# Cyan4973/FiniteStateEntropy

Hardware: NVIDIA H100
Metric: encode+decode GB/s (uncompressed) per GPU on 32 KB blocks; bit-exact vs ref (higher is better)
Workload: dtype u8

## Files before the change

finitestateentropy_b200/csrc/huf_build_dev.cuh:

```cuda
#pragma once
#include "common.cuh"
#include "fse_dev.cuh"
#include "sink_dev.cuh"

namespace fseb {

struct HNode { u32 count; u16 parent; u8 sym; u8 len; };

__device__ inline u32 d_huf_limit_depth(HNode* nd, u32 last, u32 maxBits)
{
    u32 const deepest = nd[last].len;
    if (deepest <= maxBits) return deepest;
    int debt = 0;
    u32 const unit = 1u << (deepest - maxBits);
    int n = (int)last;
    u32 const NONE = 0xF0F0F0F0u;
    u32 lastOfRank[HUF_MAX_TLOG + 2];
    while (nd[n].len > maxBits) {
        debt += (int)(unit - (1u << (deepest - nd[n].len)));
        nd[n].len = (u8)maxBits; n--;
    }
    while (nd[n].len == maxBits) n--;
    debt >>= (deepest - maxBits);
    for (u32 i = 0; i < HUF_MAX_TLOG + 2; i++) lastOfRank[i] = NONE;
    {   u32 cur = maxBits;
        for (int pos = n; pos >= 0; pos--) {
            if (nd[pos].len >= cur) continue;
            cur = nd[pos].len;
            lastOfRank[maxBits - cur] = (u32)pos;
        }
    }
    while (debt > 0) {
        u32 dec = hibit((u32)debt) + 1;
        for (; dec > 1; dec--) {
            u32 const hi = lastOfRank[dec], lo = lastOfRank[dec - 1];
            if (hi == NONE) continue;
            if (lo == NONE) break;
            if (nd[hi].count <= 2 * nd[lo].count) break;
        }
        while (dec <= HUF_MAX_TLOG && lastOfRank[dec] == NONE) dec++;
        debt -= 1 << (dec - 1);
        if (lastOfRank[dec - 1] == NONE) lastOfRank[dec - 1] = lastOfRank[dec];
        nd[lastOfRank[dec]].len++;
        if (lastOfRank[dec] == 0) lastOfRank[dec] = NONE;
        else {
            lastOfRank[dec]--;
            if (nd[lastOfRank[dec]].len != maxBits - dec) lastOfRank[dec] = NONE;
        }
    }
    while (debt < 0) {
        if (lastOfRank[1] == NONE) {
            while (nd[n].len == maxBits) n--;
            nd[n + 1].len--;
            lastOfRank[1] = (u32)(n + 1);
            debt++;
            continue;
        }
        nd[lastOfRank[1] + 1].len--;
        lastOfRank[1]++;
        debt++;
    }
    return maxBits;
}

__device__ inline u64 cta_huf_build_ctable(u32* ctable, const u32* count, u32 msv, u32 maxBits,
                                           HNode* store, u32* lenOf, u32* firstVal)
{
    int const tid = threadIdx.x;
    HNode* const nd = store + 1;
    __shared__ u32 s_ret;
    if (!maxBits) maxBits = HUF_DEF_TLOG;
    if (msv > HUF_MAX_SV) return err(E_MSV_TOO_LARGE);
    for (int i = tid; i < 2 * 256 + 2; i += blockDim.x) { HNode z; z.count = 0; z.parent = 0; z.sym = 0; z.len = 0; store[i] = z; }
    __syncthreads();
    if ((u32)tid <= msv) {
        u32 const c = count[tid];
        u32 rank = 0;
        for (u32 jj = 0; jj <= msv; jj++) { u32 const cj = count[jj]; rank += (cj > c) | ((cj == c) & (jj < (u32)tid)); }
        nd[rank].count = c; nd[rank].sym = (u8)tid;
    }
    __syncthreads();
    if (tid == 0) {
        int last = (int)msv; while (nd[last].count == 0) last--;
        int fresh = 256, leaf = last, root = fresh + leaf - 1, inner = fresh;
        nd[fresh].count = nd[leaf].count + nd[leaf - 1].count;
        nd[leaf].parent = nd[leaf - 1].parent = (u16)fresh;
        fresh++; leaf -= 2;
        for (int n = fresh; n <= root; n++) nd[n].count = 1u << 30;
        nd[-1].count = 1u << 31;
        while (fresh <= root) {
            int const a = (nd[leaf].count < nd[inner].count) ? leaf-- : inner++;
            int const b = (nd[leaf].count < nd[inner].count) ? leaf-- : inner++;
            nd[fresh].count = nd[a].count + nd[b].count;
            nd[a].parent = nd[b].parent = (u16)fresh;
            fresh++;
        }
        nd[root].len = 0;
        for (int n = root - 1; n >= 256; n--) nd[n].len = (u8)(nd[nd[n].parent].len + 1);
        for (int n = 0; n <= last; n++) nd[n].len = (u8)(nd[nd[n].parent].len + 1);
        u32 const mb = d_huf_limit_depth(nd, (u32)last, maxBits);
        s_ret = mb;
        if (mb <= HUF_MAX_TLOG) {
            u32 perLen[HUF_MAX_TLOG + 1];
            for (u32 i = 0; i <= HUF_MAX_TLOG; i++) perLen[i] = 0;
            for (int n = 0; n <= last; n++) perLen[nd[n].len]++;
            u32 v = 0;
            for (u32 i = 0; i <= HUF_MAX_TLOG; i++) firstVal[i] = 0;
            for (int n = (int)mb; n > 0; n--) { firstVal[n] = v; v = (v + perLen[n]) >> 1; }
        }
    }
    __syncthreads();
    u32 const mb = s_ret;
    if (mb > HUF_MAX_TLOG) return err(E_GENERIC);
    if ((u32)tid <= msv) lenOf[nd[tid].sym] = nd[tid].len;
    __syncthreads();
    if ((u32)tid <= msv) {
        u32 const len = lenOf[tid];
        u32 before = 0;
        for (u32 jj = 0; jj < (u32)tid; jj++) before += (lenOf[jj] == len);
        ctable[tid] = ((firstVal[len] + before) & 0xFFFF) | (len << 16);
    } else ctable[tid & 255] = 0;
    __syncthreads();
    return mb;
}

__device__ __forceinline__ void warp_sort256_desc(u32 (&key)[8], unsigned lane)
{
    #pragma unroll
    for (u32 k = 2; k <= 256; k <<= 1) {
        #pragma unroll
        for (u32 j = k >> 1; j > 0; j >>= 1) {
            if (j >= 32) {
                u32 const dj = j >> 5;
                #pragma unroll
                for (u32 i = 0; i < 8; i++) {
                    if (i & dj) continue;
                    u32 const e = i * 32;
                    bool const desc = (k == 256) || ((e & k) != 0) ;
                    u32 const lo = min(key[i], key[i | dj]), hi = max(key[i], key[i | dj]);
                    key[i] = desc ? hi : lo; key[i | dj] = desc ? lo : hi;
                }
            } else {
                #pragma unroll
                for (u32 i = 0; i < 8; i++) {
                    u32 const e = i * 32 + lane;
                    u32 const other = __shfl_xor_sync(0xFFFFFFFFu, key[i], j);
                    bool const asc = (k == 256) ? false : ((e & k) == 0);
                    bool const takeMin = ((e & j) == 0) == asc;
                    key[i] = takeMin ? min(key[i], other) : max(key[i], other);
                }
            }
        }
    }
}

__device__ inline u64 warp_huf_build_ctable(u32* ctable, const u32* count, u32 msv, u32 maxBits,
                                            HNode* store, u8* lenOf, u32* firstVal)
{
    unsigned const lane = threadIdx.x & 31u;
    HNode* const nd = store + 1;
    if (!maxBits) maxBits = HUF_DEF_TLOG;
    if (msv > HUF_MAX_SV) return err(E_MSV_TOO_LARGE);
    {
        u32 key[8];
        #pragma unroll
        for (u32 i = 0; i < 8; i++) { u32 const s = i * 32 + lane; key[i] = ((s <= msv ? count[s] : 0u) << 8) | (255u - s); }
        warp_sort256_desc(key, lane);
        u64* const z = reinterpret_cast<u64*>(store);
        #pragma unroll
        for (u32 i = 0; i < 8; i++) {
            HNode h; h.count = key[i] >> 8; h.parent = 0; h.sym = (u8)(255u - (key[i] & 0xFFu)); h.len = 0;
            nd[i * 32 + lane] = h;
        }
        if (lane == 0) z[0] = 0;
        for (u32 i = 257 + lane; i < 2 * 256 + 2; i += 32) z[i] = 0;
    }
    __syncwarp();
    u32 mb = 0; int last = 0;
    if (lane == 0) {
        last = (int)msv; while (nd[last].count == 0) last--;
        int fresh = 256, leaf = last, root = fresh + leaf - 1, inner = fresh;
        nd[fresh].count = nd[leaf].count + nd[leaf - 1].count;
        nd[leaf].parent = nd[leaf - 1].parent = (u16)fresh;
        fresh++; leaf -= 2;
        for (int n = fresh; n <= root; n++) nd[n].count = 1u << 30;
        nd[-1].count = 1u << 31;
        u32 cl = nd[leaf].count, ci = nd[inner].count;
        while (fresh <= root) {
            int a, b2; u32 ca, cb;
            if (cl < ci) { a = leaf--; ca = cl; cl = nd[leaf].count; } else { a = inner++; ca = ci; ci = nd[inner].count; }
            if (cl < ci) { b2 = leaf--; cb = cl; cl = nd[leaf].count; } else { b2 = inner++; cb = ci; ci = nd[inner].count; }
            nd[fresh].count = ca + cb;
            if (inner == fresh) ci = ca + cb;
            nd[a].parent = nd[b2].parent = (u16)fresh;
            fresh++;
        }
        nd[root].len = 0;
        for (int n = root - 1; n >= 256; n--) nd[n].len = (u8)(nd[nd[n].parent].len + 1);
    }
    last = __shfl_sync(0xFFFFFFFFu, last, 0);
    __syncwarp();
    for (int n = (int)lane; n <= last; n += 32) nd[n].len = (u8)(nd[nd[n].parent].len + 1);
    __syncwarp();
    if (lane == 0) {
        mb = d_huf_limit_depth(nd, (u32)last, maxBits);
        if (mb <= HUF_MAX_TLOG) {
            u32 perLen[HUF_MAX_TLOG + 1];
            for (u32 i = 0; i <= HUF_MAX_TLOG; i++) perLen[i] = 0;
            for (int n = 0; n <= last; n++) perLen[nd[n].len]++;
            u32 v = 0;
            for (u32 i = 0; i <= HUF_MAX_TLOG; i++) firstVal[i] = 0;
            for (int n = (int)mb; n > 0; n--) { firstVal[n] = v; v = (v + perLen[n]) >> 1; }
        }
    }
    mb = __shfl_sync(0xFFFFFFFFu, mb, 0);
    if (mb > HUF_MAX_TLOG) return err(E_GENERIC);
    if (lane < 16) firstVal[16 + lane] = 0;
    __syncwarp();
    for (u32 s = lane; s <= msv; s += 32) lenOf[nd[s].sym] = nd[s].len;
    __syncwarp();
    u32* const seen = firstVal + 16;
    for (u32 s0 = 0; s0 < 256; s0 += 32) {
        u32 const s = s0 + lane;
        u32 const len = s <= msv ? lenOf[s] : 31u;
        u32 const peers = __match_any_sync(0xFFFFFFFFu, len);
        u32 val = 0;
        if (s <= msv) val = ((firstVal[len] + seen[len] + __popc(peers & ((1u << lane) - 1))) & 0xFFFF) | (len << 16);
        __syncwarp();
        if (s <= msv && (peers >> lane) == 1u) seen[len] += __popc(peers);
        ctable[s] = val;
        __syncwarp();
    }
    return mb;
}

__device__ inline u64 d_huf_compress_weights(u8* out, u64 cap, const u8* w, u64 n, u32* wksp)
{
    unsigned* const count = wksp;
    short* const norm = (short*)(wksp + 16);
    u32* const ct = wksp + 24;
    u16* const cellSym = (u16*)(wksp + 84);
    u32* const start = wksp + 116;
    unsigned msv = HUF_MAX_TLOG, tl = 6, best = 0;
    if (n <= 1) return 0;
    for (unsigned i = 0; i <= HUF_MAX_TLOG; i++) count[i] = 0;
    for (u64 i = 0; i < n; i++) count[w[i]]++;
    while (!count[msv]) msv--;
    for (unsigned s = 0; s <= msv; s++) best = count[s] > best ? count[s] : best;
    if (best == n) return 1;
    if (best == 1) return 0;
    tl = d_optimal_tablelog(tl, n, msv, 2);
    u64 r = d_normalize(norm, tl, count, n, msv); if (is_err(r)) return r;
    r = d_write_ncount(out, cap, norm, msv, tl); if (is_err(r)) return r;
    u64 const o = r;
    d_build_ctable_serial(ct, norm, msv, tl, cellSym, start);
    r = d_fse_encode_serial(out + o, cap - o, w, n, ct);
    if (r == 0) return 0;
    return o + r;
}

__device__ inline u64 d_huf_write_ctable(u8* out, u64 cap, const u32* ctable, unsigned msv, unsigned huffLog, u32* wksp)
{
    u8* const weight = (u8*)(wksp + 160);
    if (msv > HUF_MAX_SV) return err(E_MSV_TOO_LARGE);
    for (unsigned n = 0; n < msv; n++) {
        unsigned const len = (ctable[n] >> 16) & 0xFF;
        weight[n] = (u8)(len ? huffLog + 1 - len : 0);
    }
    {   u64 const h = d_huf_compress_weights(out + 1, cap - 1, weight, msv, wksp);
        if (is_err(h)) return h;
        if ((h > 1) & (h < msv / 2)) { out[0] = (u8)h; return h + 1; }
    }
    if (msv > 128) return err(E_GENERIC);
    if (((msv + 1) / 2) + 1 > cap) return err(E_DST_TOO_SMALL);
    out[0] = (u8)(128 + (msv - 1));
    weight[msv] = 0;
    for (unsigned n = 0; n < msv; n += 2) out[(n / 2) + 1] = (u8)((weight[n] << 4) + weight[n + 1]);
    return ((msv + 1) / 2) + 1;
}

__device__ inline u64 warp_huf_compress_weights(u8* out, u64 cap, const u8* w, u32 n, u32* wksp)
{
    unsigned const lane = threadIdx.x & 31u;
    unsigned* const count = wksp;
    short* const norm = (short*)(wksp + 16);
    u32* const ct = wksp + 24;
    u16* const cellSym = (u16*)(wksp + 84);
    u32* const start = wksp + 116;
    u16* const rec = (u16*)(wksp + 224);
    if (n <= 1) return 0;
    if (lane < 16) count[lane] = 0;
    __syncwarp();
    for (u32 i = lane; i < n; i += 32) atomicAdd(&count[w[i]], 1u);
    __syncwarp();
    unsigned msv = HUF_MAX_TLOG, best = 0;
    while (!count[msv]) msv--;
    for (unsigned s = 0; s <= msv; s++) best = count[s] > best ? count[s] : best;
    if (best == n) return 1;
    if (best == 1) return 0;
    unsigned const tl = d_optimal_tablelog(6, n, msv, 2);
    u64 r = 0;
    if (lane == 0) {
        r = d_normalize(norm, tl, count, n, msv);
        if (!is_err(r)) r = d_write_ncount(out, cap, norm, msv, tl);
        if (!is_err(r)) d_build_ctable_serial(ct, norm, msv, tl, cellSym, start);
    }
    r = __shfl_sync(0xFFFFFFFFu, r, 0);
    if (is_err(r)) return r;
    u32 const o = (u32)r;
    __syncwarp();
    if (n <= 2) return 0;
    u64 const scap = cap - o;
    if (scap <= 8) return 0;
    CtView const c = ct_view(ct);
    u32 state = 0;
    if (lane < 2) {
        bool seeded = false;
        int const first = (int)(((n - 1) & 1u) == lane ? n - 1 : n - 2);
        for (int i = first; i >= 0; i -= 2) {
            u32 const sym = w[i];
            if (!seeded) { state = enc_seed(c, sym); seeded = true; rec[i] = 0; }
            else {
                u32 const nb = (state + c.tt[2 * sym + 1]) >> 16;
                rec[i] = (u16)((state & ((1u << nb) - 1)) | (nb << 8));
                state = c.next[(state >> nb) + c.tt[2 * sym]];
            }
        }
    }
    u32 const s0 = __shfl_sync(0xFFFFFFFFu, state, 0), s1 = __shfl_sync(0xFFFFFFFFu, state, 1);
    for (u32 i = o + lane; i < (u32)cap; i += 32) out[i] = 0;
    __syncwarp();
    u64 const a0 = reinterpret_cast<u64>(out + o);
    u32* const words = reinterpret_cast<u32*>(a0 & ~3ull);
    u32 const limitWords = (u32)(((a0 & 3) + scap + 3) / 4);
    u32 running = 8 * (u32)(a0 & 3);
    u32 const bit0 = running;
    u32 const R = n + 3;
    for (u32 k0 = 0; k0 < R; k0 += 32) {
        u32 const k = k0 + lane;
        u32 e = 0;
        if (k < n) e = rec[n - 1 - k];
        else if (k == n) e = (s1 & ((1u << tl) - 1)) | (tl << 8);
        else if (k == n + 1) e = (s0 & ((1u << tl) - 1)) | (tl << 8);
        else if (k == n + 2) e = 1u | (1u << 8);
        u32 const nb = e >> 8, val = e & 0xFF;
        u32 incl = nb;
        #pragma unroll
        for (int d = 1; d < 32; d <<= 1) { u32 const t = __shfl_up_sync(0xFFFFFFFFu, incl, d); if (lane >= (unsigned)d) incl += t; }
        u32 const sum = __shfl_sync(0xFFFFFFFFu, incl, 31);
        if (nb) {
            u32 const off = running + incl - nb;
            u32 const wi = off >> 5, sh = off & 31;
            if (wi < limitWords) atomicOr(&words[wi], val << sh);
            if (sh + nb > 32 && wi + 1 < limitWords) atomicOr(&words[wi + 1], val >> (32 - sh));
        }
        running += sum;
    }
    __syncwarp();
    u32 const totalBits = running - bit0;
    if ((u64)(totalBits >> 3) >= scap - 8) return 0;
    return (u64)o + ((totalBits + 7) >> 3);
}

__device__ inline u64 warp_huf_write_ctable(u8* out, u64 cap, const u32* ctable, unsigned msv, unsigned huffLog, u32* wksp)
{
    unsigned const lane = threadIdx.x & 31u;
    u8* const weight = (u8*)(wksp + 160);
    if (msv > HUF_MAX_SV) return err(E_MSV_TOO_LARGE);
    for (unsigned n = lane; n < msv; n += 32) {
        unsigned const len = (ctable[n] >> 16) & 0xFF;
        weight[n] = (u8)(len ? huffLog + 1 - len : 0);
    }
    __syncwarp();
    {   u64 const h = warp_huf_compress_weights(out + 1, cap - 1, weight, msv, wksp);
        if (is_err(h)) return h;
        if ((h > 1) & (h < msv / 2)) { if (lane == 0) out[0] = (u8)h; __syncwarp(); return h + 1; }
    }
    if (msv > 128) return err(E_GENERIC);
    if (((msv + 1) / 2) + 1 > cap) return err(E_DST_TOO_SMALL);
    __syncwarp();
    if (lane == 0) { out[0] = (u8)(128 + (msv - 1)); weight[msv] = 0; }
    __syncwarp();
    for (unsigned n = 2 * lane; n < msv; n += 64) out[(n / 2) + 1] = (u8)((weight[n] << 4) + weight[n + 1]);
    __syncwarp();
    return ((msv + 1) / 2) + 1;
}

}
```

finitestateentropy_b200/csrc/huf_encode.cu:

```cuda
#include <cstdlib>
#include <mutex>
#include <vector>
#include "common.cuh"
#include "launch_util.cuh"
#include "fse_dev.cuh"
#include "sink_dev.cuh"
#include "huf_build_dev.cuh"

namespace fseb {
namespace hufe {

constexpr unsigned FULL = 0xFFFFFFFFu;

struct __align__(16) Plan {
    u32 ctable[256];
    u8  header[136];
    u32 hSize;
    u32 state;
    u32 total;
    u32 streamOff[4];
    u32 streamBytes[4];
};

constexpr int PLAN_WARPS = 8;
struct PlanWarp {
    u32   count4[4][256];
    u32   count[256];
    HNode nodes[2 * 256 + 2];
    u32   ctable[256];
    u32   firstVal[32];
    u8    lenOf[256];
    alignas(4) u8 header[136];
};
static_assert(sizeof(HNode) * (2 * 256 + 2) >= 384 * sizeof(u32), "header scratch must fit in the node array");
__device__ __forceinline__ u32 seg_count(const PlanWarp& w, u32 k, u32 i) { return w.count4[k][i]; }

__device__ __forceinline__ void warp_hist_range(u32* cnt, const u8* s, u32 begin, u32 end, unsigned lane)
{
    u32 i = begin;
    u32 const head = min(end, (u32)((begin + 15) & ~15u));
    bool const vec = ((reinterpret_cast<u64>(s) & 15) == 0);
    if (vec) {
        for (u32 k = i + lane; k < head; k += 32) atomicAdd(&cnt[s[k]], 1u);
        i = head;
        u32 const nvec = (end - i) / 16;
        const uint4* const gv = reinterpret_cast<const uint4*>(s + i);
        for (u32 v0 = 0; v0 < nvec; v0 += 128) {
            uint4 x[4];
            #pragma unroll
            for (int h = 0; h < 4; h++) { u32 const vi = v0 + 32 * h + lane; x[h] = (vi < nvec) ? __ldg(gv + vi) : make_uint4(0, 0, 0, 0); }
            #pragma unroll
            for (int h = 0; h < 4; h++) {
                if (v0 + 32 * h + lane >= nvec) continue;
                u32 const wd[4] = { x[h].x, x[h].y, x[h].z, x[h].w };
                #pragma unroll
                for (int k = 0; k < 4; k++) {
                    u32 const y = wd[k];
                    atomicAdd(&cnt[y & 0xFF], 1u); atomicAdd(&cnt[__byte_perm(y, 0, 0x4441)], 1u);
                    atomicAdd(&cnt[__byte_perm(y, 0, 0x4442)], 1u); atomicAdd(&cnt[y >> 24], 1u);
                }
            }
        }
        i += nvec * 16;
    }
    for (u32 k = i + lane; k < end; k += 32) atomicAdd(&cnt[s[k]], 1u);
}

__device__ __forceinline__ void warp_hist4_pipelined(u32 (*count4)[256], const u8* s, u32 n, u32 seg, unsigned lane)
{
    const uint4* const gv = reinterpret_cast<const uint4*>(s) + lane;
    u32 const B = n / 2048, perSeg = seg / 2048;
    auto load = [&](uint4 (&x)[4], u32 b) {
        #pragma unroll
        for (int h = 0; h < 4; h++) x[h] = __ldg(gv + b * 128 + 32 * h);
    };
    auto count = [&](const uint4 (&x)[4], u32 b) {
        u32* const cnt = count4[b / perSeg];
        #pragma unroll
        for (int h = 0; h < 4; h++) {
            u32 const wd[4] = { x[h].x, x[h].y, x[h].z, x[h].w };
            #pragma unroll
            for (int k = 0; k < 4; k++) {
                u32 const y = wd[k];
                atomicAdd(&cnt[y & 0xFF], 1u); atomicAdd(&cnt[__byte_perm(y, 0, 0x4441)], 1u);
                atomicAdd(&cnt[__byte_perm(y, 0, 0x4442)], 1u); atomicAdd(&cnt[y >> 24], 1u);
            }
        }
    };
    uint4 xa[4], xb[4];
    load(xa, 0);
    #pragma unroll 1
    for (u32 b = 0; b < B; b += 2) {
        if (b + 1 < B) load(xb, b + 1);
        count(xa, b);
        if (b + 2 < B) load(xa, b + 2);
        if (b + 1 < B) count(xb, b + 1);
    }
}

__global__ void __launch_bounds__(32 * PLAN_WARPS)
huf_plan_kernel(BatchGeom g, u8* __restrict__ cbuf, u64* __restrict__ csizes, const u8* __restrict__ src,
                unsigned msvReq, unsigned tlogReq, Plan* __restrict__ plans, int serialHeader)
{
    extern __shared__ __align__(16) unsigned char smem_raw[];
    PlanWarp& w = reinterpret_cast<PlanWarp*>(smem_raw)[threadIdx.x >> 5];
    unsigned const lane = threadIdx.x & 31u;
    u32 const b = blockIdx.x * PLAN_WARPS + (threadIdx.x >> 5);
    if (b >= g.nBlocks) return;
    u32 const n = block_len(g, b);
    const u8* const s = src + (u64)b * g.blockSize;
    u8* const d = cbuf + (u64)b * g.slot;
    u64 const cap = g.slot;
    Plan& P = plans[b];
#define FSEB_FINAL(v) do { if (lane == 0) { P.state = 1; csizes[b] = (v); } return; } while (0)

    if (!n) FSEB_FINAL(0);
    if (!cap) FSEB_FINAL(0);
    if (n > HUF_BLOCK_MAX) FSEB_FINAL(err(E_SRC_WRONG));
    if (tlogReq > HUF_MAX_TLOG) FSEB_FINAL(err(E_TLOG_TOO_LARGE));
    if (msvReq > HUF_MAX_SV) FSEB_FINAL(err(E_MSV_TOO_LARGE));
    unsigned const msvDecl = msvReq ? msvReq : HUF_MAX_SV;
    unsigned huffLog = tlogReq ? tlogReq : HUF_DEF_TLOG;

    u32 const seg = (n + 3) / 4;
    for (u32 i = lane; i < 4 * 256; i += 32) (&w.count4[0][0])[i] = 0;
    __syncwarp();
    if ((reinterpret_cast<u64>(s) & 15) == 0 && seg % 2048 == 0 && n == 4 * seg) warp_hist4_pipelined(w.count4, s, n, seg, lane);
    else {
        #pragma unroll 1
        for (u32 k = 0; k < 4; k++) {
            u32 const beg = min(k * seg, n), end = (k < 3) ? min((k + 1) * seg, n) : n;
            warp_hist_range(w.count4[k], s, beg, end, lane);
        }
    }
    __syncwarp();
    u32 top = 0, best = 0;
    for (u32 i = lane; i < 256; i += 32) {
        u32 const c = seg_count(w, 0, i) + seg_count(w, 1, i) + seg_count(w, 2, i) + seg_count(w, 3, i);
        w.count[i] = c;
        if (c) top = i; best = c > best ? c : best;
    }
    #pragma unroll
    for (int dlt = 16; dlt; dlt >>= 1) { top = max(top, __shfl_xor_sync(FULL, top, dlt)); best = max(best, __shfl_xor_sync(FULL, best, dlt)); }
    __syncwarp();
    if (msvDecl < 255 && top > msvDecl) FSEB_FINAL(err(E_MSV_TOO_SMALL));
    if (best == n) { if (lane == 0) d[0] = s[0]; FSEB_FINAL(1); }
    if (best <= (n >> 7) + 4) FSEB_FINAL(0);
    u32 const msv = top;

    huffLog = d_optimal_tablelog(huffLog, n, msv, 1);
    {   u64 const mb = warp_huf_build_ctable(w.ctable, w.count, msv, huffLog, w.nodes, w.lenOf, w.firstVal);
        if (is_err(mb)) FSEB_FINAL(mb);
        huffLog = (u32)mb;
    }
    __syncwarp();
    u32* const wksp = reinterpret_cast<u32*>(w.nodes);
    u64 hs = 0;
    if (serialHeader) { if (lane == 0) hs = d_huf_write_ctable(w.header, cap < sizeof(w.header) ? cap : sizeof(w.header), w.ctable, msv, huffLog, wksp); hs = __shfl_sync(FULL, hs, 0); }
    else hs = warp_huf_write_ctable(w.header, cap < sizeof(w.header) ? cap : sizeof(w.header), w.ctable, msv, huffLog, wksp);
    if (is_err(hs)) FSEB_FINAL(hs);
    if (hs + 12 >= n) FSEB_FINAL(0);
    u64 const capLeft = cap - hs;
    if (capLeft < 6 + 1 + 1 + 1 + 8 || n < 12) FSEB_FINAL(0);
    u32 bits[4];
    #pragma unroll
    for (int k = 0; k < 4; k++) {
        u32 acc = 0;
        for (u32 i = lane; i <= msv; i += 32) acc += seg_count(w, k, i) * (w.ctable[i] >> 16);
        #pragma unroll
        for (int dlt = 16; dlt; dlt >>= 1) acc += __shfl_xor_sync(FULL, acc, dlt);
        bits[k] = acc;
    }
    u64 op = 6; bool fits = true;
    u32 offs[4], lens[4];
    #pragma unroll
    for (int t = 0; t < 4; t++) {
        u64 const capk = capLeft - op;
        u64 const tot = (u64)bits[t] + 1;
        if (fits && (capk <= 8 || (tot >> 3) >= capk - 8)) fits = false;
        offs[t] = (u32)(hs + op); lens[t] = (u32)((tot + 7) >> 3);
        op += lens[t];
    }
    u64 const total = hs + op;
    if (!fits || total >= (u64)n - 1) FSEB_FINAL(0);
    __syncwarp();
    for (u32 i = lane; i < 256; i += 32) P.ctable[i] = w.ctable[i];
    for (u32 i = lane; i < (u32)hs; i += 32) P.header[i] = w.header[i];
    if (lane < 4) { P.streamOff[lane] = offs[lane]; P.streamBytes[lane] = lens[lane]; }
    if (lane == 0) { P.hSize = (u32)hs; P.state = 0; P.total = (u32)total; csizes[b] = total; }
#undef FSEB_FINAL
}

constexpr int THREADS = 128;

__device__ __noinline__ void store_piece_exact(u32* gw, u32 j, uint4 v, u32 a0, u32 endByte)
{
    u32 const wd[4] = { v.x, v.y, v.z, v.w };
    u8* const pb = reinterpret_cast<u8*>(gw + j);
    for (u32 t = 0; t < 16; t++) { u32 const at = 4 * j + t; if (at >= a0 && at < endByte) pb[t] = (u8)(wd[t >> 2] >> (8 * (t & 3))); }
}

__global__ void __launch_bounds__(THREADS)
huf_emit_kernel(BatchGeom g, u8* __restrict__ cbuf, const u8* __restrict__ src, const Plan* __restrict__ plans, const u32* __restrict__ sharedCT)
{
    constexpr u32 W = 512;
    __shared__ u32 ctab[256];
    constexpr u32 WP = W + 4;
    __shared__ __align__(16) u32 winAll[4 * WP];
    int const tid = threadIdx.x;
    unsigned const lane = tid & 31u; int const k = tid >> 5;
    u32 const b = blockIdx.x;
    const Plan& P = plans[b];
    if (P.state != 0) return;
    u32 const n = block_len(g, b);
    const u8* const s = src + (u64)b * g.blockSize;
    u8* const d = cbuf + (u64)b * g.slot;
    u32 const hSize = P.hSize, total = P.total;

    {   const u32* const ct = sharedCT ? sharedCT : P.ctable;
        u32 const c0 = ct[tid], c1 = ct[tid + 128];
        ctab[tid] = (c0 >> 16) | (c0 << 8 & 0xFFFF00u); ctab[tid + 128] = (c1 >> 16) | (c1 << 8 & 0xFFFF00u);
    }
    for (u32 i = tid; i < 4 * WP; i += THREADS) winAll[i] = 0;
    for (u32 i = tid; i < hSize; i += THREADS) d[i] = P.header[i];
    if (tid < 3) { u32 const v = P.streamBytes[tid]; d[hSize + 2 * tid] = (u8)v; d[hSize + 2 * tid + 1] = (u8)(v >> 8); }
    __syncthreads();
    {
        u32 const seg = (n + 3) / 4;
        int const segBeg = (int)(k * seg);
        int const segEnd = (k < 3) ? (int)((k + 1) * seg) : (int)n;
        u32 sTab = (u32)__cvta_generic_to_shared(ctab);
        asm volatile("mov.u32 %0, %0;" : "+r"(sTab));
        u32* const win = winAll + k * WP;
        u32 sWin = (u32)__cvta_generic_to_shared(win);
        asm volatile("mov.u32 %0, %0;" : "+r"(sWin));
        u8* const gstart = d + P.streamOff[k];
        u32 const a0 = (u32)(reinterpret_cast<u64>(gstart) & 15);
        u32* const gw = reinterpret_cast<u32*>(gstart - a0);
        u32 const sBytes = (k < 3) ? P.streamBytes[k] : total - P.streamOff[3];
        u32 const endByte = a0 + sBytes;
        u32 bitpos = 8u * a0;
        u32 flushed = 0;
// ... 199 lines not shown
    for (int t = 0; t < 4; t++) {
        u64 const capk = cap - op;
        u64 const tot = (u64)bits[t] + 1;
        if (fits && (capk <= 8 || (tot >> 3) >= capk - 8)) fits = false;
        offs[t] = (u32)op; lens[t] = (u32)((tot + 7) >> 3);
        op += lens[t];
    }
    if (!fits) { if (lane == 0) { P.state = 1; csizes[b] = 0; } return; }
    if (lane < 4) { P.streamOff[lane] = offs[lane]; P.streamBytes[lane] = lens[lane]; }
    if (lane == 0) { P.hSize = 0; P.state = 0; P.total = (u32)op; csizes[b] = op; }
}

}

cudaError_t launch_huf_encode_using_ctable(const BatchGeom& g, void* cbuf, u64* csizes, const void* src, const u32* dCTable, cudaStream_t stream)
{
    if (g.nBlocks == 0) return cudaSuccess;
    cudaError_t e;
    hufe::Plan* const plans = (hufe::Plan*)stream_scratch(2, stream, sizeof(hufe::Plan) * (size_t)g.nBlocks, &e);
    if (e != cudaSuccess) return e;
    unsigned const grid = (g.nBlocks + hufe::PLAN_WARPS - 1) / hufe::PLAN_WARPS;
    hufe::huf_sizes_kernel<<<grid, 32 * hufe::PLAN_WARPS, 0, stream>>>(g, csizes, (const u8*)src, dCTable, plans);
    hufe::huf_emit_kernel<<<g.nBlocks, hufe::THREADS, 0, stream>>>(g, (u8*)cbuf, (const u8*)src, plans, dCTable);
    return cudaGetLastError();
}

cudaError_t launch_huf_encode(const BatchGeom& g, void* cbuf, u64* csizes, const void* src,
                              unsigned msv, unsigned tlog, cudaStream_t stream)
{
    if (g.nBlocks == 0) return cudaSuccess;
    cudaError_t e;
    hufe::Plan* plans = nullptr;
    static int asyncScratch = -1;
    if (asyncScratch < 0) { const char* const v = getenv("FSEB200_SCRATCH_ASYNC"); asyncScratch = (v && atoi(v) == 1) ? 1 : 0; }
    size_t const need = sizeof(hufe::Plan) * (size_t)g.nBlocks;
    if (asyncScratch) e = cudaMallocAsync((void**)&plans, need, stream);
    else {
        struct Slot { int dev; cudaStream_t s; void* p; size_t cap; };
        static std::mutex mu; static std::vector<Slot> slots;
        std::lock_guard<std::mutex> lock(mu);
        int dev = 0; cudaGetDevice(&dev);
        Slot* hit = nullptr;
        for (auto& sl : slots) if (sl.s == stream && sl.dev == dev) { hit = &sl; break; }
        if (!hit) { slots.push_back(Slot{ dev, stream, nullptr, 0 }); hit = &slots.back(); }
        e = cudaSuccess;
        if (hit->cap < need) {
            if (hit->p) { cudaStreamSynchronize(stream); cudaFree(hit->p); hit->p = nullptr; hit->cap = 0; }
            e = cudaMalloc(&hit->p, need);
            if (e == cudaSuccess) hit->cap = need;
        }
        plans = (hufe::Plan*)hit->p;
    }
    if (e != cudaSuccess) return e;
    static int serialHeader = -1;
    if (serialHeader < 0) { const char* const v = getenv("FSEB200_HUF_SERIAL_HEADER"); serialHeader = (v && atoi(v) == 1) ? 1 : 0; }
    static u32 const subBatch = [] { const char* const v = getenv("FSEB200_HUF_ENC_SUBBATCH"); long n = v ? atol(v) : 0; return (u32)(n < 0 ? 0 : n); }();
    size_t const smem = sizeof(hufe::PlanWarp) * hufe::PLAN_WARPS;
    static SmemOptIn optin;
    e = optin.ensure(hufe::huf_plan_kernel, current_device(), (int)smem);
    if (e != cudaSuccess) return e;
    u32 const step = (subBatch && subBatch < g.nBlocks) ? subBatch : g.nBlocks;
    for (u32 b0 = 0; b0 < g.nBlocks; b0 += step) {
        BatchGeom gs = g;
        gs.nBlocks = (g.nBlocks - b0 < step) ? g.nBlocks - b0 : step;
        u64 const off = (u64)b0 * g.blockSize;
        u64 const span = (u64)gs.nBlocks * g.blockSize;
        gs.total = (g.total - off < span) ? g.total - off : span;
        u8* const cb = (u8*)cbuf + (u64)b0 * g.slot; const u8* const sp = (const u8*)src + off;
        unsigned const grid = (gs.nBlocks + hufe::PLAN_WARPS - 1) / hufe::PLAN_WARPS;
        hufe::huf_plan_kernel<<<grid, 32 * hufe::PLAN_WARPS, smem, stream>>>(gs, cb, csizes + b0, sp, msv, tlog, plans + b0, serialHeader);
        hufe::huf_emit_kernel<<<gs.nBlocks, hufe::THREADS, 0, stream>>>(gs, cb, sp, plans + b0, nullptr);
    }
    e = cudaGetLastError();
    cudaError_t const e2 = asyncScratch ? cudaFreeAsync(plans, stream) : cudaSuccess;
    return e != cudaSuccess ? e : e2;
}

}
```

Baseline: 363.7.

## Build Huffman tables for 32 blocks per CTA with one lane per block

Restructures the Huffman plan kernel so each CTA takes 32 blocks. Warps first compute histograms and sort symbols. Then warp 0 builds the tree, limits depth, assigns codes and writes headers with one lane per block, on packed column-major node words in shared memory. This replaces the old single-lane-per-warp serial tree build, which left 31 lanes idle. Segment counts are now stored in the plan so the later stage can size the streams. The change adds a larger shared-memory footprint and a packed 24-bit count/8-bit tag format, and it removes the serial-header option.

```diff
diff --git a/finitestateentropy_b200/csrc/huf_build_dev.cuh b/finitestateentropy_b200/csrc/huf_build_dev.cuh
--- a/finitestateentropy_b200/csrc/huf_build_dev.cuh
+++ b/finitestateentropy_b200/csrc/huf_build_dev.cuh
@@ -7,26 +7,40 @@
 
 struct HNode { u32 count; u16 parent; u8 sym; u8 len; };
 
-__device__ inline u32 d_huf_limit_depth(HNode* nd, u32 last, u32 maxBits)
-{
-    u32 const deepest = nd[last].len;
+struct HNodeView {
+    HNode* p;
+    __device__ u32 count(int i) const { return p[i].count; }
+    __device__ u32 len(int i) const { return p[i].len; }
+    __device__ void set_len(int i, u32 v) const { p[i].len = (u8)v; }
+};
+struct PackedNodeView {
+    u32* p; int stride;
+    __device__ u32 count(int i) const { return p[i * stride] & 0xFFFFFFu; }
+    __device__ u32 len(int i) const { return p[i * stride] >> 24; }
+    __device__ void set_len(int i, u32 v) const { u32& x = p[i * stride]; x = (x & 0xFFFFFFu) | (v << 24); }
+};
+
+template <class Nodes>
+__device__ inline u32 d_huf_limit_depth(Nodes nd, u32 last, u32 maxBits)
+{
+    u32 const deepest = nd.len(last);
     if (deepest <= maxBits) return deepest;
     int debt = 0;
     u32 const unit = 1u << (deepest - maxBits);
     int n = (int)last;
     u32 const NONE = 0xF0F0F0F0u;
     u32 lastOfRank[HUF_MAX_TLOG + 2];
-    while (nd[n].len > maxBits) {
-        debt += (int)(unit - (1u << (deepest - nd[n].len)));
-        nd[n].len = (u8)maxBits; n--;
-    }
-    while (nd[n].len == maxBits) n--;
+    while (nd.len(n) > maxBits) {
+        debt += (int)(unit - (1u << (deepest - nd.len(n))));
+        nd.set_len(n, maxBits); n--;
+    }
+    while (nd.len(n) == maxBits) n--;
     debt >>= (deepest - maxBits);
     for (u32 i = 0; i < HUF_MAX_TLOG + 2; i++) lastOfRank[i] = NONE;
     {   u32 cur = maxBits;
         for (int pos = n; pos >= 0; pos--) {
-            if (nd[pos].len >= cur) continue;
-            cur = nd[pos].len;
+            if (nd.len(pos) >= cur) continue;
+            cur = nd.len(pos);
             lastOfRank[maxBits - cur] = (u32)pos;
         }
     }
@@ -36,27 +50,27 @@
             u32 const hi = lastOfRank[dec], lo = lastOfRank[dec - 1];
             if (hi == NONE) continue;
             if (lo == NONE) break;
-            if (nd[hi].count <= 2 * nd[lo].count) break;
+            if (nd.count(hi) <= 2 * nd.count(lo)) break;
         }
         while (dec <= HUF_MAX_TLOG && lastOfRank[dec] == NONE) dec++;
         debt -= 1 << (dec - 1);
         if (lastOfRank[dec - 1] == NONE) lastOfRank[dec - 1] = lastOfRank[dec];
-        nd[lastOfRank[dec]].len++;
+        nd.set_len(lastOfRank[dec], nd.len(lastOfRank[dec]) + 1);
         if (lastOfRank[dec] == 0) lastOfRank[dec] = NONE;
         else {
             lastOfRank[dec]--;
-            if (nd[lastOfRank[dec]].len != maxBits - dec) lastOfRank[dec] = NONE;
+            if (nd.len(lastOfRank[dec]) != maxBits - dec) lastOfRank[dec] = NONE;
         }
     }
     while (debt < 0) {
         if (lastOfRank[1] == NONE) {
-            while (nd[n].len == maxBits) n--;
-            nd[n + 1].len--;
+            while (nd.len(n) == maxBits) n--;
+            nd.set_len(n + 1, nd.len(n + 1) - 1);
             lastOfRank[1] = (u32)(n + 1);
             debt++;
             continue;
         }
-        nd[lastOfRank[1] + 1].len--;
+        nd.set_len(lastOfRank[1] + 1, nd.len(lastOfRank[1] + 1) - 1);
         lastOfRank[1]++;
         debt++;
     }
@@ -98,7 +112,7 @@
         nd[root].len = 0;
         for (int n = root - 1; n >= 256; n--) nd[n].len = (u8)(nd[nd[n].parent].len + 1);
         for (int n = 0; n <= last; n++) nd[n].len = (u8)(nd[nd[n].parent].len + 1);
-        u32 const mb = d_huf_limit_depth(nd, (u32)last, maxBits);
+        u32 const mb = d_huf_limit_depth(HNodeView{ nd }, (u32)last, maxBits);
         s_ret = mb;
         if (mb <= HUF_MAX_TLOG) {
             u32 perLen[HUF_MAX_TLOG + 1];
@@ -154,86 +168,6 @@
     }
 }
 
-__device__ inline u64 warp_huf_build_ctable(u32* ctable, const u32* count, u32 msv, u32 maxBits,
-                                            HNode* store, u8* lenOf, u32* firstVal)
-{
-    unsigned const lane = threadIdx.x & 31u;
-    HNode* const nd = store + 1;
-    if (!maxBits) maxBits = HUF_DEF_TLOG;
-    if (msv > HUF_MAX_SV) return err(E_MSV_TOO_LARGE);
-    {
-        u32 key[8];
-        #pragma unroll
-        for (u32 i = 0; i < 8; i++) { u32 const s = i * 32 + lane; key[i] = ((s <= msv ? count[s] : 0u) << 8) | (255u - s); }
-        warp_sort256_desc(key, lane);
-        u64* const z = reinterpret_cast<u64*>(store);
-        #pragma unroll
-        for (u32 i = 0; i < 8; i++) {
-            HNode h; h.count = key[i] >> 8; h.parent = 0; h.sym = (u8)(255u - (key[i] & 0xFFu)); h.len = 0;
-            nd[i * 32 + lane] = h;
-        }
-        if (lane == 0) z[0] = 0;
-        for (u32 i = 257 + lane; i < 2 * 256 + 2; i += 32) z[i] = 0;
-    }
-    __syncwarp();
-    u32 mb = 0; int last = 0;
-    if (lane == 0) {
-        last = (int)msv; while (nd[last].count == 0) last--;
-        int fresh = 256, leaf = last, root = fresh + leaf - 1, inner = fresh;
-        nd[fresh].count = nd[leaf].count + nd[leaf - 1].count;
-        nd[leaf].parent = nd[leaf - 1].parent = (u16)fresh;
-        fresh++; leaf -= 2;
-        for (int n = fresh; n <= root; n++) nd[n].count = 1u << 30;
-        nd[-1].count = 1u << 31;
-        u32 cl = nd[leaf].count, ci = nd[inner].count;
-        while (fresh <= root) {
-            int a, b2; u32 ca, cb;
-            if (cl < ci) { a = leaf--; ca = cl; cl = nd[leaf].count; } else { a = inner++; ca = ci; ci = nd[inner].count; }
-            if (cl < ci) { b2 = leaf--; cb = cl; cl = nd[leaf].count; } else { b2 = inner++; cb = ci; ci = nd[inner].count; }
-            nd[fresh].count = ca + cb;
-            if (inner == fresh) ci = ca + cb;
-            nd[a].parent = nd[b2].parent = (u16)fresh;
-            fresh++;
-        }
-        nd[root].len = 0;
-        for (int n = root - 1; n >= 256; n--) nd[n].len = (u8)(nd[nd[n].parent].len + 1);
-    }
-    last = __shfl_sync(0xFFFFFFFFu, last, 0);
-    __syncwarp();
-    for (int n = (int)lane; n <= last; n += 32) nd[n].len = (u8)(nd[nd[n].parent].len + 1);
-    __syncwarp();
-    if (lane == 0) {
-        mb = d_huf_limit_depth(nd, (u32)last, maxBits);
-        if (mb <= HUF_MAX_TLOG) {
-            u32 perLen[HUF_MAX_TLOG + 1];
-            for (u32 i = 0; i <= HUF_MAX_TLOG; i++) perLen[i] = 0;
-            for (int n = 0; n <= last; n++) perLen[nd[n].len]++;
-            u32 v = 0;
-            for (u32 i = 0; i <= HUF_MAX_TLOG; i++) firstVal[i] = 0;
-            for (int n = (int)mb; n > 0; n--) { firstVal[n] = v; v = (v + perLen[n]) >> 1; }
-        }
-    }
-    mb = __shfl_sync(0xFFFFFFFFu, mb, 0);
-    if (mb > HUF_MAX_TLOG) return err(E_GENERIC);
-    if (lane < 16) firstVal[16 + lane] = 0;
-    __syncwarp();
-    for (u32 s = lane; s <= msv; s += 32) lenOf[nd[s].sym] = nd[s].len;
-    __syncwarp();
-    u32* const seen = firstVal + 16;
-    for (u32 s0 = 0; s0 < 256; s0 += 32) {
-        u32 const s = s0 + lane;
-        u32 const len = s <= msv ? lenOf[s] : 31u;
-        u32 const peers = __match_any_sync(0xFFFFFFFFu, len);
-        u32 val = 0;
-        if (s <= msv) val = ((firstVal[len] + seen[len] + __popc(peers & ((1u << lane) - 1))) & 0xFFFF) | (len << 16);
-        __syncwarp();
-        if (s <= msv && (peers >> lane) == 1u) seen[len] += __popc(peers);
-        ctable[s] = val;
-        __syncwarp();
-    }
-    return mb;
-}
-
 __device__ inline u64 d_huf_compress_weights(u8* out, u64 cap, const u8* w, u64 n, u32* wksp)
 {
     unsigned* const count = wksp;
@@ -259,7 +193,8 @@
     return o + r;
 }
 
-__device__ inline u64 d_huf_write_ctable(u8* out, u64 cap, const u32* ctable, unsigned msv, unsigned huffLog, u32* wksp)
+template <class CTable>
+__device__ inline u64 d_huf_write_ctable(u8* out, u64 cap, CTable ctable, unsigned msv, unsigned huffLog, u32* wksp)
 {
     u8* const weight = (u8*)(wksp + 160);
     if (msv > HUF_MAX_SV) return err(E_MSV_TOO_LARGE);
@@ -279,111 +214,4 @@
     return ((msv + 1) / 2) + 1;
 }
 
-__device__ inline u64 warp_huf_compress_weights(u8* out, u64 cap, const u8* w, u32 n, u32* wksp)
-{
-    unsigned const lane = threadIdx.x & 31u;
-    unsigned* const count = wksp;
-    short* const norm = (short*)(wksp + 16);
-    u32* const ct = wksp + 24;
-    u16* const cellSym = (u16*)(wksp + 84);
-    u32* const start = wksp + 116;
-    u16* const rec = (u16*)(wksp + 224);
-    if (n <= 1) return 0;
-    if (lane < 16) count[lane] = 0;
-    __syncwarp();
-    for (u32 i = lane; i < n; i += 32) atomicAdd(&count[w[i]], 1u);
-    __syncwarp();
-    unsigned msv = HUF_MAX_TLOG, best = 0;
-    while (!count[msv]) msv--;
-    for (unsigned s = 0; s <= msv; s++) best = count[s] > best ? count[s] : best;
-    if (best == n) return 1;
-    if (best == 1) return 0;
-    unsigned const tl = d_optimal_tablelog(6, n, msv, 2);
-    u64 r = 0;
-    if (lane == 0) {
-        r = d_normalize(norm, tl, count, n, msv);
-        if (!is_err(r)) r = d_write_ncount(out, cap, norm, msv, tl);
-        if (!is_err(r)) d_build_ctable_serial(ct, norm, msv, tl, cellSym, start);
-    }
-    r = __shfl_sync(0xFFFFFFFFu, r, 0);
-    if (is_err(r)) return r;
-    u32 const o = (u32)r;
-    __syncwarp();
-    if (n <= 2) return 0;
-    u64 const scap = cap - o;
-    if (scap <= 8) return 0;
-    CtView const c = ct_view(ct);
-    u32 state = 0;
-    if (lane < 2) {
-        bool seeded = false;
-        int const first = (int)(((n - 1) & 1u) == lane ? n - 1 : n - 2);
-        for (int i = first; i >= 0; i -= 2) {
-            u32 const sym = w[i];
-            if (!seeded) { state = enc_seed(c, sym); seeded = true; rec[i] = 0; }
-            else {
-                u32 const nb = (state + c.tt[2 * sym + 1]) >> 16;
-                rec[i] = (u16)((state & ((1u << nb) - 1)) | (nb << 8));
-                state = c.next[(state >> nb) + c.tt[2 * sym]];
-            }
-        }
-    }
-    u32 const s0 = __shfl_sync(0xFFFFFFFFu, state, 0), s1 = __shfl_sync(0xFFFFFFFFu, state, 1);
-    for (u32 i = o + lane; i < (u32)cap; i += 32) out[i] = 0;
-    __syncwarp();
-    u64 const a0 = reinterpret_cast<u64>(out + o);
-    u32* const words = reinterpret_cast<u32*>(a0 & ~3ull);
-    u32 const limitWords = (u32)(((a0 & 3) + scap + 3) / 4);
-    u32 running = 8 * (u32)(a0 & 3);
-    u32 const bit0 = running;
-    u32 const R = n + 3;
-    for (u32 k0 = 0; k0 < R; k0 += 32) {
-        u32 const k = k0 + lane;
-        u32 e = 0;
-        if (k < n) e = rec[n - 1 - k];
-        else if (k == n) e = (s1 & ((1u << tl) - 1)) | (tl << 8);
-        else if (k == n + 1) e = (s0 & ((1u << tl) - 1)) | (tl << 8);
-        else if (k == n + 2) e = 1u | (1u << 8);
-        u32 const nb = e >> 8, val = e & 0xFF;
-        u32 incl = nb;
-        #pragma unroll
-        for (int d = 1; d < 32; d <<= 1) { u32 const t = __shfl_up_sync(0xFFFFFFFFu, incl, d); if (lane >= (unsigned)d) incl += t; }
-        u32 const sum = __shfl_sync(0xFFFFFFFFu, incl, 31);
-        if (nb) {
-            u32 const off = running + incl - nb;
-            u32 const wi = off >> 5, sh = off & 31;
-            if (wi < limitWords) atomicOr(&words[wi], val << sh);
-            if (sh + nb > 32 && wi + 1 < limitWords) atomicOr(&words[wi + 1], val >> (32 - sh));
-        }
-        running += sum;
-    }
-    __syncwarp();
-    u32 const totalBits = running - bit0;
-    if ((u64)(totalBits >> 3) >= scap - 8) return 0;
-    return (u64)o + ((totalBits + 7) >> 3);
-}
-
-__device__ inline u64 warp_huf_write_ctable(u8* out, u64 cap, const u32* ctable, unsigned msv, unsigned huffLog, u32* wksp)
-{
-    unsigned const lane = threadIdx.x & 31u;
-    u8* const weight = (u8*)(wksp + 160);
-    if (msv > HUF_MAX_SV) return err(E_MSV_TOO_LARGE);
-    for (unsigned n = lane; n < msv; n += 32) {
-        unsigned const len = (ctable[n] >> 16) & 0xFF;
-        weight[n] = (u8)(len ? huffLog + 1 - len : 0);
-    }
-    __syncwarp();
-    {   u64 const h = warp_huf_compress_weights(out + 1, cap - 1, weight, msv, wksp);
-        if (is_err(h)) return h;
-        if ((h > 1) & (h < msv / 2)) { if (lane == 0) out[0] = (u8)h; __syncwarp(); return h + 1; }
-    }
-    if (msv > 128) return err(E_GENERIC);
-    if (((msv + 1) / 2) + 1 > cap) return err(E_DST_TOO_SMALL);
-    __syncwarp();
-    if (lane == 0) { out[0] = (u8)(128 + (msv - 1)); weight[msv] = 0; }
-    __syncwarp();
-    for (unsigned n = 2 * lane; n < msv; n += 64) out[(n / 2) + 1] = (u8)((weight[n] << 4) + weight[n + 1]);
-    __syncwarp();
-    return ((msv + 1) / 2) + 1;
-}
-
-}
+}
diff --git a/finitestateentropy_b200/csrc/huf_encode.cu b/finitestateentropy_b200/csrc/huf_encode.cu
--- a/finitestateentropy_b200/csrc/huf_encode.cu
+++ b/finitestateentropy_b200/csrc/huf_encode.cu
@@ -20,20 +20,28 @@
     u32 total;
     u32 streamOff[4];
     u32 streamBytes[4];
+    u16 segCount[4][256];
 };
 
 constexpr int PLAN_WARPS = 8;
-struct PlanWarp {
-    u32   count4[4][256];
-    u32   count[256];
-    HNode nodes[2 * 256 + 2];
-    u32   ctable[256];
-    u32   firstVal[32];
-    u8    lenOf[256];
-    alignas(4) u8 header[136];
+constexpr u32 GROUP = 32;
+constexpr u32 HDR_STRIDE = 34 + 224 + 1;
+constexpr u32 CT_ROW = HDR_STRIDE;
+constexpr u32 ROWS = CT_ROW + 256;
+constexpr u32 NODE_END = 0x7FFFFFFFu, LEAF_END = 0xFFFFFFFFu;
+struct PlanCta {
+    u32 nd[ROWS][GROUP];
+    u8  sym[256][GROUP];
+    u64 res[GROUP];
+    u16 msv[GROUP];
+    u8  last[GROUP];
+    u8  tlog[GROUP];
+    u8  live[GROUP];
 };
-static_assert(sizeof(HNode) * (2 * 256 + 2) >= 384 * sizeof(u32), "header scratch must fit in the node array");
-__device__ __forceinline__ u32 seg_count(const PlanWarp& w, u32 k, u32 i) { return w.count4[k][i]; }
+static_assert(ROWS >= 1 + 256 + PLAN_WARPS * 4 * 256 / GROUP, "segment histograms must fit in the rows above the leaves");
+static_assert(ROWS >= 1 + 511 && CT_ROW >= 1 + 256, "node rows");
+static_assert(HUF_BLOCK_MAX < (1u << 24), "node counts share a word with an 8-bit parent / length");
+static_assert(sizeof(PlanCta) <= 76 * 1024, "three CTAs per SM");
 
 __device__ __forceinline__ void warp_hist_range(u32* cnt, const u8* s, u32 begin, u32 end, unsigned lane)
 {
@@ -98,96 +106,178 @@
     }
 }
 
-__global__ void __launch_bounds__(32 * PLAN_WARPS)
+__global__ void __launch_bounds__(32 * PLAN_WARPS, 3)
 huf_plan_kernel(BatchGeom g, u8* __restrict__ cbuf, u64* __restrict__ csizes, const u8* __restrict__ src,
-                unsigned msvReq, unsigned tlogReq, Plan* __restrict__ plans, int serialHeader)
+                unsigned msvReq, unsigned tlogReq, Plan* __restrict__ plans)
 {
     extern __shared__ __align__(16) unsigned char smem_raw[];
-    PlanWarp& w = reinterpret_cast<PlanWarp*>(smem_raw)[threadIdx.x >> 5];
-    unsigned const lane = threadIdx.x & 31u;
-    u32 const b = blockIdx.x * PLAN_WARPS + (threadIdx.x >> 5);
-    if (b >= g.nBlocks) return;
-    u32 const n = block_len(g, b);
-    const u8* const s = src + (u64)b * g.blockSize;
-    u8* const d = cbuf + (u64)b * g.slot;
+    PlanCta& S = *reinterpret_cast<PlanCta*>(smem_raw);
+    unsigned const lane = threadIdx.x & 31u, warp = threadIdx.x >> 5;
+    u32 const b0 = blockIdx.x * GROUP;
     u64 const cap = g.slot;
-    Plan& P = plans[b];
-#define FSEB_FINAL(v) do { if (lane == 0) { P.state = 1; csizes[b] = (v); } return; } while (0)
-
-    if (!n) FSEB_FINAL(0);
-    if (!cap) FSEB_FINAL(0);
-    if (n > HUF_BLOCK_MAX) FSEB_FINAL(err(E_SRC_WRONG));
-    if (tlogReq > HUF_MAX_TLOG) FSEB_FINAL(err(E_TLOG_TOO_LARGE));
-    if (msvReq > HUF_MAX_SV) FSEB_FINAL(err(E_MSV_TOO_LARGE));
-    unsigned const msvDecl = msvReq ? msvReq : HUF_MAX_SV;
-    unsigned huffLog = tlogReq ? tlogReq : HUF_DEF_TLOG;
-
-    u32 const seg = (n + 3) / 4;
-    for (u32 i = lane; i < 4 * 256; i += 32) (&w.count4[0][0])[i] = 0;
-    __syncwarp();
-    if ((reinterpret_cast<u64>(s) & 15) == 0 && seg % 2048 == 0 && n == 4 * seg) warp_hist4_pipelined(w.count4, s, n, seg, lane);
-    else {
-        #pragma unroll 1
-        for (u32 k = 0; k < 4; k++) {
-            u32 const beg = min(k * seg, n), end = (k < 3) ? min((k + 1) * seg, n) : n;
-            warp_hist_range(w.count4[k], s, beg, end, lane);
-        }
-    }
-    __syncwarp();
-    u32 top = 0, best = 0;
-    for (u32 i = lane; i < 256; i += 32) {
-        u32 const c = seg_count(w, 0, i) + seg_count(w, 1, i) + seg_count(w, 2, i) + seg_count(w, 3, i);
-        w.count[i] = c;
-        if (c) top = i; best = c > best ? c : best;
-    }
-    #pragma unroll
-    for (int dlt = 16; dlt; dlt >>= 1) { top = max(top, __shfl_xor_sync(FULL, top, dlt)); best = max(best, __shfl_xor_sync(FULL, best, dlt)); }
-    __syncwarp();
-    if (msvDecl < 255 && top > msvDecl) FSEB_FINAL(err(E_MSV_TOO_SMALL));
-    if (best == n) { if (lane == 0) d[0] = s[0]; FSEB_FINAL(1); }
-    if (best <= (n >> 7) + 4) FSEB_FINAL(0);
-    u32 const msv = top;
-
-    huffLog = d_optimal_tablelog(huffLog, n, msv, 1);
-    {   u64 const mb = warp_huf_build_ctable(w.ctable, w.count, msv, huffLog, w.nodes, w.lenOf, w.firstVal);
-        if (is_err(mb)) FSEB_FINAL(mb);
-        huffLog = (u32)mb;
-    }
-    __syncwarp();
-    u32* const wksp = reinterpret_cast<u32*>(w.nodes);
-    u64 hs = 0;
-    if (serialHeader) { if (lane == 0) hs = d_huf_write_ctable(w.header, cap < sizeof(w.header) ? cap : sizeof(w.header), w.ctable, msv, huffLog, wksp); hs = __shfl_sync(FULL, hs, 0); }
-    else hs = warp_huf_write_ctable(w.header, cap < sizeof(w.header) ? cap : sizeof(w.header), w.ctable, msv, huffLog, wksp);
-    if (is_err(hs)) FSEB_FINAL(hs);
-    if (hs + 12 >= n) FSEB_FINAL(0);
-    u64 const capLeft = cap - hs;
-    if (capLeft < 6 + 1 + 1 + 1 + 8 || n < 12) FSEB_FINAL(0);
-    u32 bits[4];
-    #pragma unroll
-    for (int k = 0; k < 4; k++) {
-        u32 acc = 0;
-        for (u32 i = lane; i <= msv; i += 32) acc += seg_count(w, k, i) * (w.ctable[i] >> 16);
-        #pragma unroll
-        for (int dlt = 16; dlt; dlt >>= 1) acc += __shfl_xor_sync(FULL, acc, dlt);
-        bits[k] = acc;
-    }
-    u64 op = 6; bool fits = true;
-    u32 offs[4], lens[4];
-    #pragma unroll
-    for (int t = 0; t < 4; t++) {
-        u64 const capk = capLeft - op;
-        u64 const tot = (u64)bits[t] + 1;
-        if (fits && (capk <= 8 || (tot >> 3) >= capk - 8)) fits = false;
-        offs[t] = (u32)(hs + op); lens[t] = (u32)((tot + 7) >> 3);
-        op += lens[t];
-    }
-    u64 const total = hs + op;
-    if (!fits || total >= (u64)n - 1) FSEB_FINAL(0);
-    __syncwarp();
-    for (u32 i = lane; i < 256; i += 32) P.ctable[i] = w.ctable[i];
-    for (u32 i = lane; i < (u32)hs; i += 32) P.header[i] = w.header[i];
-    if (lane < 4) { P.streamOff[lane] = offs[lane]; P.streamBytes[lane] = lens[lane]; }
-    if (lane == 0) { P.hSize = (u32)hs; P.state = 0; P.total = (u32)total; csizes[b] = total; }
+#define FSEB_FINAL(v) { if (lane == 0) { P.state = 1; csizes[b] = (v); S.live[c] = 0; } continue; }
+
+    u32 (*const count4)[256] = reinterpret_cast<u32 (*)[256]>(&S.nd[257][0] + warp * 4 * 256);
+    #pragma unroll 1
+    for (u32 c = warp; c < GROUP; c += PLAN_WARPS) {
+        __syncwarp();
+        u32 const b = b0 + c;
+        if (b >= g.nBlocks) { if (lane == 0) S.live[c] = 0; continue; }
+        u32 const n = block_len(g, b);
+        const u8* const s = src + (u64)b * g.blockSize;
+        Plan& P = plans[b];
+        if (!n) FSEB_FINAL(0);
+        if (!cap) FSEB_FINAL(0);
+        if (n > HUF_BLOCK_MAX) FSEB_FINAL(err(E_SRC_WRONG));
+        if (tlogReq > HUF_MAX_TLOG) FSEB_FINAL(err(E_TLOG_TOO_LARGE));
+        if (msvReq > HUF_MAX_SV) FSEB_FINAL(err(E_MSV_TOO_LARGE));
+        unsigned const msvDecl = msvReq ? msvReq : HUF_MAX_SV;
+
+        u32 const seg = (n + 3) / 4;
+        for (u32 i = lane; i < 4 * 256; i += 32) (&count4[0][0])[i] = 0;
+        __syncwarp();
+        if ((reinterpret_cast<u64>(s) & 15) == 0 && seg % 2048 == 0 && n == 4 * seg) warp_hist4_pipelined(count4, s, n, seg, lane);
+        else {
+            #pragma unroll 1
+            for (u32 k = 0; k < 4; k++) {
+                u32 const beg = min(k * seg, n), end = (k < 3) ? min((k + 1) * seg, n) : n;
+                warp_hist_range(count4[k], s, beg, end, lane);
+            }
+        }
+        __syncwarp();
+        u32 cnt[8], top = 0, best = 0;
+        #pragma unroll
+        for (u32 i = 0; i < 8; i++) {
+            u32 const sy = i * 32 + lane;
+            cnt[i] = count4[0][sy] + count4[1][sy] + count4[2][sy] + count4[3][sy];
+            if (cnt[i]) top = sy;
+            best = max(best, cnt[i]);
+        }
+        #pragma unroll
+        for (int dlt = 16; dlt; dlt >>= 1) { top = max(top, __shfl_xor_sync(FULL, top, dlt)); best = max(best, __shfl_xor_sync(FULL, best, dlt)); }
+        if (msvDecl < 255 && top > msvDecl) FSEB_FINAL(err(E_MSV_TOO_SMALL));
+        if (best == n) { if (lane == 0) cbuf[(u64)b * g.slot] = s[0]; FSEB_FINAL(1); }
+        if (best <= (n >> 7) + 4) FSEB_FINAL(0);
+        u32 const msv = top;
+        #pragma unroll
+        for (u32 k = 0; k < 4; k++)
+            #pragma unroll
+            for (u32 i = 0; i < 8; i++) P.segCount[k][i * 32 + lane] = (u16)count4[k][i * 32 + lane];
+        u32 key[8], nnz = 0;
+        #pragma unroll
+        for (u32 i = 0; i < 8; i++) { u32 const sy = i * 32 + lane; key[i] = ((sy <= msv ? cnt[i] : 0u) << 8) | (255u - sy); nnz += __popc(__ballot_sync(FULL, cnt[i] != 0)); }
+        warp_sort256_desc(key, lane);
+        #pragma unroll
+        for (u32 i = 0; i < 8; i++) {
+            u32 const r = i * 32 + lane;
+            if (r <= msv) { S.nd[1 + r][c] = key[i] >> 8; S.sym[r][c] = (u8)(255u - (key[i] & 0xFFu)); }
+        }
+        if (lane == 0) {
+            S.nd[0][c] = 0;
+            S.msv[c] = (u16)msv; S.last[c] = (u8)(nnz - 1); S.live[c] = 1;
+            S.tlog[c] = (u8)d_optimal_tablelog(tlogReq ? tlogReq : HUF_DEF_TLOG, n, msv, 1);
+        }
+    }
+    __syncthreads();
+
+    if (warp == 0) {
+        u32 const c = lane;
+        bool const live = S.live[c];
+        u32 const msv = S.msv[c];
+        u32* const col = &S.nd[1][c];
+        auto at = [&](int i) -> u32& { return col[i * (int)GROUP]; };
+        u32* const ct = &S.nd[CT_ROW][c];
+        u64 res = 0;
+        if (live) {
+            int const last = S.last[c];
+            int fresh = 256, leaf = last, inner = fresh;
+            int const root = fresh + leaf - 1;
+            {   u32 const x = at(leaf), y = at(leaf - 1);
+                at(fresh) = x + y;
+                fresh++; leaf -= 2;
+            }
+            u32 cl = leaf >= 0 ? at(leaf) : LEAF_END, ci = at(inner);
+            while (fresh <= root) {
+                int a, bb; u32 ca, cb;
+                if (cl < ci) { a = leaf--; ca = cl; cl = leaf >= 0 ? at(leaf) : LEAF_END; } else { a = inner++; ca = ci; ci = inner < fresh ? at(inner) : NODE_END; }
+                if (cl < ci) { bb = leaf--; cb = cl; cl = leaf >= 0 ? at(leaf) : LEAF_END; } else { bb = inner++; cb = ci; ci = inner < fresh ? at(inner) : NODE_END; }
+                u32 const sum = ca + cb;
+                at(fresh) = sum;
+                if (inner == fresh) ci = sum;
+                u32 const tag = (u32)(fresh - 256) << 24;
+                at(a) = ca | tag; at(bb) = cb | tag;
+                fresh++;
+            }
+            at(root) &= 0xFFFFFFu;
+            for (int m = root - 1; m >= 256; m--) { u32 const v = at(m); at(m) = (v & 0xFFFFFFu) | (((at(256 + (int)(v >> 24)) >> 24) + 1) << 24); }
+            for (int m = 0; m <= last; m++) { u32 const v = at(m); at(m) = (v & 0xFFFFFFu) | (((at(256 + (int)(v >> 24)) >> 24) + 1) << 24); }
+            u32 const mb = d_huf_limit_depth(PackedNodeView{ col, (int)GROUP }, (u32)last, S.tlog[c]);
+            if (mb > HUF_MAX_TLOG) res = err(E_GENERIC);
+            else {
+                u32 perLen[HUF_MAX_TLOG + 1], nextVal[HUF_MAX_TLOG + 1];
+                for (u32 i = 0; i <= HUF_MAX_TLOG; i++) { perLen[i] = 0; nextVal[i] = 0; }
+                for (int m = 0; m <= last; m++) perLen[at(m) >> 24]++;
+                u32 v = 0;
+                for (int m = (int)mb; m > 0; m--) { nextVal[m] = v; v = (v + perLen[m]) >> 1; }
+                for (u32 r = 0; r <= msv; r++) ct[S.sym[r][c] * GROUP] = (int)r <= last ? at((int)r) >> 24 : 0u;
+                for (u32 sy = 0; sy <= msv; sy++) { u32 const len = ct[sy * GROUP]; ct[sy * GROUP] = (nextVal[len]++ & 0xFFFF) | (len << 16); }
+                S.tlog[c] = (u8)mb;
+            }
+        }
+        __syncwarp();
+        if (live && !is_err(res)) {
+            u32* const area = &S.nd[0][0] + c * HDR_STRIDE;
+            struct Col { const u32* p; __device__ u32 operator[](u32 i) const { return p[i * GROUP]; } };
+            res = d_huf_write_ctable(reinterpret_cast<u8*>(area), cap < 136 ? cap : 136, Col{ ct }, msv, S.tlog[c], area + 34);
+        }
+        S.res[c] = res;
+    }
+    __syncthreads();
+
+    #pragma unroll 1
+    for (u32 c = warp; c < GROUP; c += PLAN_WARPS) {
+        if (!S.live[c]) continue;
+        u32 const b = b0 + c;
+        u32 const n = block_len(g, b);
+        Plan& P = plans[b];
+        u64 const hs = S.res[c];
+        if (is_err(hs)) FSEB_FINAL(hs);
+        if (hs + 12 >= n) FSEB_FINAL(0);
+        u64 const capLeft = cap - hs;
+        if (capLeft < 6 + 1 + 1 + 1 + 8 || n < 12) FSEB_FINAL(0);
+        u32 const msv = S.msv[c];
+        u32 cell[8];
+        #pragma unroll
+        for (u32 i = 0; i < 8; i++) cell[i] = (i * 32 + lane <= msv) ? S.nd[CT_ROW + i * 32 + lane][c] : 0u;
+        u32 bits[4];
+        #pragma unroll
+        for (int k = 0; k < 4; k++) {
+            u32 acc = 0;
+            #pragma unroll
+            for (u32 i = 0; i < 8; i++) acc += (u32)P.segCount[k][i * 32 + lane] * (cell[i] >> 16);
+            #pragma unroll
+            for (int dlt = 16; dlt; dlt >>= 1) acc += __shfl_xor_sync(FULL, acc, dlt);
+            bits[k] = acc;
+        }
+        u64 op = 6; bool fits = true;
+        u32 offs[4], lens[4];
+        #pragma unroll
+        for (int t = 0; t < 4; t++) {
+            u64 const capk = capLeft - op;
+            u64 const tot = (u64)bits[t] + 1;
+            if (fits && (capk <= 8 || (tot >> 3) >= capk - 8)) fits = false;
+            offs[t] = (u32)(hs + op); lens[t] = (u32)((tot + 7) >> 3);
+            op += lens[t];
+        }
+        u64 const total = hs + op;
+        if (!fits || total >= (u64)n - 1) FSEB_FINAL(0);
+        #pragma unroll
+        for (u32 i = 0; i < 8; i++) P.ctable[i * 32 + lane] = cell[i];
+        const u8* const hdr = reinterpret_cast<const u8*>(&S.nd[0][0] + c * HDR_STRIDE);
+        for (u32 i = lane; i < (u32)hs; i += 32) P.header[i] = hdr[i];
+        if (lane < 4) { P.streamOff[lane] = offs[lane]; P.streamBytes[lane] = lens[lane]; }
+        if (lane == 0) { P.hSize = (u32)hs; P.state = 0; P.total = (u32)total; csizes[b] = total; }
+    }
 #undef FSEB_FINAL
 }
 
@@ -493,10 +583,8 @@
         plans = (hufe::Plan*)hit->p;
     }
     if (e != cudaSuccess) return e;
-    static int serialHeader = -1;
-    if (serialHeader < 0) { const char* const v = getenv("FSEB200_HUF_SERIAL_HEADER"); serialHeader = (v && atoi(v) == 1) ? 1 : 0; }
     static u32 const subBatch = [] { const char* const v = getenv("FSEB200_HUF_ENC_SUBBATCH"); long n = v ? atol(v) : 0; return (u32)(n < 0 ? 0 : n); }();
-    size_t const smem = sizeof(hufe::PlanWarp) * hufe::PLAN_WARPS;
+    size_t const smem = sizeof(hufe::PlanCta);
     static SmemOptIn optin;
     e = optin.ensure(hufe::huf_plan_kernel, current_device(), (int)smem);
     if (e != cudaSuccess) return e;
@@ -508,8 +596,8 @@
         u64 const span = (u64)gs.nBlocks * g.blockSize;
         gs.total = (g.total - off < span) ? g.total - off : span;
         u8* const cb = (u8*)cbuf + (u64)b0 * g.slot; const u8* const sp = (const u8*)src + off;
-        unsigned const grid = (gs.nBlocks + hufe::PLAN_WARPS - 1) / hufe::PLAN_WARPS;
-        hufe::huf_plan_kernel<<<grid, 32 * hufe::PLAN_WARPS, smem, stream>>>(gs, cb, csizes + b0, sp, msv, tlog, plans + b0, serialHeader);
+        unsigned const grid = (gs.nBlocks + hufe::GROUP - 1) / hufe::GROUP;
+        hufe::huf_plan_kernel<<<grid, 32 * hufe::PLAN_WARPS, smem, stream>>>(gs, cb, csizes + b0, sp, msv, tlog, plans + b0);
         hufe::huf_emit_kernel<<<gs.nBlocks, hufe::THREADS, 0, stream>>>(gs, cb, sp, plans + b0, nullptr);
     }
     e = cudaGetLastError();
```

Result: faster. 396.5 (median of 6 runs) (+9.0%).
